# wyf-ACCEPT/BackToReality

Hardware: NVIDIA B200
Metric: Pointnet2Backbone fwd+bwd scenes/sec @40k pts (higher is better)
Workload: dtype tf32 fwd / bf16 bwd operands, f32 accumulate

## Files before the change

backtoreality_b200/csrc/mlp_bwd.cu:

```cuda
#include <cuda_bf16.h>

#include "mlp_common.cuh"

namespace b2r {
using namespace mlp;
namespace {

constexpr int kBwdWarps = 12;
constexpr int kBwdThreads = kBwdWarps * 32;

struct BwdArgs {
  int B, N, NP, NS, Cin, Cout, mode, top;
  const float *xyz, *new_xyz, *feat_t;
  const int *idx;
  float radius;
  int normalize_xyz;
  const float *z_prev, *scale_prev, *shift_prev;
  const void *w_image;
  const float *dz;
  const float *gr, *z;
  const float *dysel;
  const int *asel;
  const float *coef_a, *coef_b, *coef_c;
  float *dW;
  float *gr_prev;
  double *stats_prev;
  float *g_feat_t, *g_xyz, *g_new_xyz;
  int do_dgrad;
  int Kp, KA, WA, Cout_pad, num_tiles;
  int ch8_shift;
  int ns_shift;
  const int *cidx, *ccen, *cmeta;
};

__host__ __device__ inline int packed_k16(int Cin, int gather) {
  if (!gather) return (Cin + 7) & ~7;
  return ((Cin - 3 + 7) & ~7) + 8;
}

struct BwdSmem {
  uint32_t w_off, w_bytes, x_off[2], dz_off[2], x_bytes, dz_bytes, coef_off, scale_off, idx_off,
      cen_off, meta_off, route_off, flush_off, bar_off, total;
};
__host__ __device__ inline BwdSmem bwd_smem_layout(int Kp, int KA, int WA, int Cout, int Cout_pad,
                                                   int NT, int top, int cmp = 0) {
  BwdSmem s;
  s.w_off = 0;
  s.w_bytes = (uint32_t)Cout_pad * WA * 128u;
  s.x_bytes = (uint32_t)NT * KA * 128u;
  s.dz_bytes = (uint32_t)NT * (Cout_pad >> 6) * 128u;
  uint32_t o = s.w_bytes;
  for (int st = 0; st < 2; ++st) {
    s.x_off[st] = o;
    o += s.x_bytes;
    s.dz_off[st] = o;
    o += s.dz_bytes;
  }
  s.coef_off = o;
  s.scale_off = s.coef_off + 3u * Cout * 4u;
  s.idx_off = s.scale_off + 2u * Kp * 4u;
  s.cen_off = s.idx_off + 4u * (uint32_t)NT * 4u;
  s.meta_off = s.cen_off + (cmp ? 4u * (uint32_t)NT * 4u : 0u);
  s.route_off = (s.meta_off + (cmp ? 32u : 0u) + 15u) & ~15u;
  s.flush_off = s.route_off +
                (top ? 4u * (uint32_t)(NT / (cmp ? 8 : 16)) * Cout_pad * 4u : 0u);
  const uint32_t flush_bytes = 8u * 32u * 33u * 4u;
  if (cmp && 2u * (s.x_bytes + s.dz_bytes) >= flush_bytes) {
    s.bar_off = s.flush_off;
    s.flush_off = s.x_off[0];
  } else {
    s.bar_off = s.flush_off + flush_bytes;
  }
  s.total = s.bar_off + 13 * 8 + 16 + 1024;
  return s;
}

__device__ __forceinline__ uint32_t bf_off(int row, int chunk, int rows) {
  const int a = chunk >> 3, c = chunk & 7, g = row >> 3, r8 = row & 7;
  return (uint32_t)(((a * (rows >> 3) + g) << 10) + (r8 << 7) + ((c ^ r8) << 4));
}
__host__ __device__ constexpr uint32_t idesc_bf16(int n, int a_mn, int b_mn) {
  return (1u << 4) | (1u << 7) | (1u << 10) | ((uint32_t)a_mn << 15) | ((uint32_t)b_mn << 16) |
         ((uint32_t)(n >> 3) << 17) | ((128u >> 4) << 24);
}
__device__ __forceinline__ void umma_bf16(uint32_t d_tmem, uint64_t a_desc, uint64_t b_desc,
                                          uint32_t idesc, uint32_t accumulate) {
  asm volatile(
      "{\n\t"
      ".reg .pred p;\n\t"
      "setp.ne.b32 p, %4, 0;\n\t"
      "tcgen05.mma.cta_group::1.kind::f16 [%0], %1, %2, %3, p;\n\t"
      "}" ::"r"(d_tmem),
      "l"(a_desc), "l"(b_desc), "r"(idesc), "r"(accumulate)
      : "memory");
}
__device__ __forceinline__ void mbar_arrive(uint32_t bar) {
  asm volatile("mbarrier.arrive.shared::cta.b64 _, [%0];" ::"r"(bar) : "memory");
}
__device__ __forceinline__ uint32_t pack_bf16(float lo, float hi) {
  const __nv_bfloat162 v = __floats2bfloat162_rn(lo, hi);
  return *reinterpret_cast<const uint32_t *>(&v);
}
template <int N>
__device__ __forceinline__ void bar_named(int id) {
  asm volatile("bar.sync %0, %1;" ::"r"(id), "n"(N));
}

__global__ void pack_weight_bf16_kernel(const float *__restrict__ w, int Cout, int Cin, int gather,
                                        int Kp, int Cout_pad, int WA,
                                        __nv_bfloat16 *__restrict__ image) {
  const long long total = (long long)Cout_pad * WA * 64;
  for (long long e = (long long)blockIdx.x * blockDim.x + threadIdx.x; e < total;
       e += (long long)gridDim.x * blockDim.x) {
    const int co = (int)(e / (WA * 64)), kp = (int)(e % (WA * 64));
    float v = 0.f;
    if (co < Cout && kp < Kp) {
      int k = -1;
      if (gather) {
        const int C = Cin - 3, Cf8 = (C + 7) & ~7;
        if (kp < C) k = 3 + kp;
        else if (kp >= Cf8 && kp < Cf8 + 3) k = kp - Cf8;
      } else if (kp < Cin) {
        k = kp;
      }
      if (k >= 0) v = w[(size_t)co * Cin + k];
    }
    image[(bf_off(co, kp >> 3, Cout_pad) >> 1) + (kp & 7)] = __float2bfloat16_rn(v);
  }
}

template <int NT, int EW, int MODE, int TOP, bool CMP>
__global__ void __launch_bounds__(kBwdThreads, 1) sa_layer_bwd_kernel(const BwdArgs a) {
  constexpr int kMode = MODE;
  constexpr bool kTop = TOP != 0;
  constexpr int kRC = CMP ? NT / 8 : NT / 16;
  constexpr int kEpiThreads = EW * 32, kProdThreads = (kBwdWarps - 1 - EW) * 32;
  auto bar_epi = [] { bar_named<kEpiThreads>(1); };
  auto bar_prod = [] { bar_named<kProdThreads>(2); };
  extern __shared__ __align__(1024) uint8_t smem_raw[];
  uint8_t *base = reinterpret_cast<uint8_t *>((reinterpret_cast<uintptr_t>(smem_raw) + 1023) &
                                              ~(uintptr_t)1023);
  const BwdSmem L = bwd_smem_layout(a.Kp, a.KA, a.WA, a.Cout, a.Cout_pad, NT, kTop, CMP ? 1 : 0);
  uint8_t *s_w = base + L.w_off;
  float *s_ca = reinterpret_cast<float *>(base + L.coef_off);
  float *s_cb = s_ca + a.Cout;
  float *s_cc = s_cb + a.Cout;
  float *s_scale = reinterpret_cast<float *>(base + L.scale_off);
  float *s_shift = s_scale + a.Kp;
  int *s_idx4 = reinterpret_cast<int *>(base + L.idx_off);
  int *s_cen4 = reinterpret_cast<int *>(base + L.cen_off);
  int *s_meta = reinterpret_cast<int *>(base + L.meta_off);
  float *s_dy = reinterpret_cast<float *>(base + L.route_off);
  int *s_as = reinterpret_cast<int *>(s_dy + 2 * kRC * a.Cout_pad);
  uint64_t *s_bar = reinterpret_cast<uint64_t *>(base + L.bar_off);
  uint32_t *s_tmem = reinterpret_cast<uint32_t *>(s_bar + 13);
  auto bar = [&](int i) { return smem_u32(&s_bar[i]); };

  const int tid = threadIdx.x, warp = tid >> 5, lane = tid & 31;
  const int KA = a.KA;
  const int MTp = (KA + 1) >> 1;
  const int MTl = a.Cout_pad >> 7;
  constexpr int NCH = NT / 32;
  const bool has_coef = a.dz == nullptr;
  const int w12 = ((kTop && MTl > (a.do_dgrad ? MTp : 0)) ? MTl : (a.do_dgrad ? MTp : 0)) * NT;
  const uint32_t d3_col0 = 2u * (uint32_t)w12;
  constexpr uint32_t kTmemCols = 512;
  const long long per_scene = (long long)a.NP * a.NS;
  const int C = a.Cin - 3, Cf8 = (C + 7) & ~7;
  int num_tiles = a.num_tiles;
  if constexpr (CMP) {
    num_tiles = __ldg(a.cmeta + 8) / NT;
    if (tid < 8) s_meta[tid] = __ldg(a.cmeta + tid);
  }

  if (tid == 0) {
    for (int i = 0; i < 13; ++i)
      mbar_init(bar(i), (i == 0 || i == 1) ? (uint32_t)(kProdThreads / 32)
                        : (i == 10 || i == 11) ? (uint32_t)EW : 1u);
    asm volatile("fence.mbarrier_init.release.cluster;" ::: "memory");
  }
  if (warp == EW) tmem_alloc(smem_u32(s_tmem), kTmemCols);
  {
    const uint32_t zb = 2u * (L.x_bytes + L.dz_bytes);
    for (uint32_t i = tid * 16; i < zb; i += kBwdThreads * 16)
      *reinterpret_cast<uint4 *>(base + L.x_off[0] + i) = make_uint4(0, 0, 0, 0);
  }
  if (kMode == 1)
    for (int i = tid; i < a.Cin; i += kBwdThreads) {
      s_scale[i] = a.scale_prev[i];
      s_shift[i] = a.shift_prev[i];
    }
  if (has_coef)
    for (int i = tid; i < a.Cout; i += kBwdThreads) {
      s_ca[i] = a.coef_a[i];
      s_cb[i] = a.coef_b[i];
      s_cc[i] = a.coef_c[i];
    }
  fence_async_smem();
  tc_fence_before();
  __syncthreads();
  tc_fence_after();
  const uint32_t tmem_base = *s_tmem;
  const bool need_w = kTop || a.do_dgrad;
  if (tid == 0 && need_w) {
    mbar_expect_tx(bar(12), L.w_bytes);
    bulk_g2s(smem_u32(s_w), a.w_image, L.w_bytes, bar(12));
  }
  const int grid = (int)gridDim.x;

  if (warp > EW) {
    const int ptid = tid - (kEpiThreads + 32);
    const int CH8 = a.Cout >> 3;
    const int ch8s = (CH8 & (CH8 - 1)) == 0 ? 31 - __clz(CH8) : -1;
    const int CHx = a.Cin >> 3;
    const int chxs = (CHx > 0 && (CHx & (CHx - 1)) == 0) ? 31 - __clz(CHx) : -1;
    int nidx = 0, ncen = 0;
    for (int k = 0, tile = blockIdx.x; tile < num_tiles; tile += grid, ++k) {
      const int s = k & 1, n = k >> 1;
      mbar_wait(bar(2 + s), (uint32_t)((n & 1) ^ 1));
      const long long pos0 = (long long)tile * NT;
      uint8_t *sx = base + L.x_off[s], *sdz = base + L.dz_off[s];
      int *s_idx = s_idx4 + (k & 3) * NT;
      int *s_cen = s_cen4 + (k & 3) * NT;
      TileClass tc{};
      int p64 = 0;
      if constexpr (CMP) {
        tc = tile_class(s_meta, pos0, a.NS);
        p64 = (int)(pos0 & 63);
      }
      if (ptid == 0 && tile + 2 * grid < num_tiles) {
        const size_t pn = (size_t)(pos0 + 2ll * grid * NT);
        if (!kTop) {
          if (!has_coef) prefetch_l2(a.dz + pn * a.Cout, (uint32_t)NT * a.Cout * 4u);
          else {
            prefetch_l2(a.gr + pn * a.Cout, (uint32_t)NT * a.Cout * 4u);
            prefetch_l2(a.z + pn * a.Cout, (uint32_t)NT * a.Cout * 4u);
          }
        }
        if (kMode == 1) prefetch_l2(a.z_prev + pn * a.Cin, (uint32_t)NT * a.Cin * 4u);
      }
      if (!kTop) {
        const int total = NT * CH8;
        const size_t o0 = (size_t)pos0 * a.Cout;
        for (int i0 = ptid; i0 < total; i0 += kProdThreads * 4) {
          float4 g[4][2], zz[4][2];
#pragma unroll
          for (int u = 0; u < 4; ++u) {
            const int i = i0 + u * kProdThreads;
            if (i < total) {
              if (!has_coef) {
                const float4 *p = reinterpret_cast<const float4 *>(a.dz + o0) + 2 * i;
                g[u][0] = __ldg(p); g[u][1] = __ldg(p + 1);
              } else {
                const float4 *p = reinterpret_cast<const float4 *>(a.gr + o0) + 2 * i;
                const float4 *qz = reinterpret_cast<const float4 *>(a.z + o0) + 2 * i;
                g[u][0] = __ldg(p); g[u][1] = __ldg(p + 1);
                zz[u][0] = __ldg(qz); zz[u][1] = __ldg(qz + 1);
              }
            }
          }
#pragma unroll
          for (int u = 0; u < 4; ++u) {
            const int i = i0 + u * kProdThreads;
            if (i < total) {
              const int row = ch8s >= 0 ? (i >> ch8s) : (i / CH8), ch = i - row * CH8;
              float v[8] = {g[u][0].x, g[u][0].y, g[u][0].z, g[u][0].w,
                            g[u][1].x, g[u][1].y, g[u][1].z, g[u][1].w};
              if (has_coef) {
                const float zv[8] = {zz[u][0].x, zz[u][0].y, zz[u][0].z, zz[u][0].w,
                                     zz[u][1].x, zz[u][1].y, zz[u][1].z, zz[u][1].w};
                float ca8[8], cb8[8], cc8[8];
                *reinterpret_cast<float4 *>(ca8) = *reinterpret_cast<const float4 *>(s_ca + ch * 8);
                *reinterpret_cast<float4 *>(ca8 + 4) = *reinterpret_cast<const float4 *>(s_ca + ch * 8 + 4);
                *reinterpret_cast<float4 *>(cb8) = *reinterpret_cast<const float4 *>(s_cb + ch * 8);
                *reinterpret_cast<float4 *>(cb8 + 4) = *reinterpret_cast<const float4 *>(s_cb + ch * 8 + 4);
                *reinterpret_cast<float4 *>(cc8) = *reinterpret_cast<const float4 *>(s_cc + ch * 8);
                *reinterpret_cast<float4 *>(cc8 + 4) = *reinterpret_cast<const float4 *>(s_cc + ch * 8 + 4);
                if constexpr (CMP) {
                  const float wgt = row < tc.live
                                        ? ((((p64 + row) & (tc.ns - 1)) == 0) ? 1.f + tc.wx : 1.f)
                                        : 0.f;
#pragma unroll
                  for (int e = 0; e < 8; ++e)
                    v[e] = fmaf(ca8[e], v[e], wgt * fmaf(cb8[e], zv[e], cc8[e]));
                } else {
#pragma unroll
                  for (int e = 0; e < 8; ++e) v[e] = fmaf(ca8[e], v[e], fmaf(cb8[e], zv[e], cc8[e]));
                }
              }
              *reinterpret_cast<uint4 *>(sdz + bf_off(row, ch, NT)) =
                  make_uint4(pack_bf16(v[0], v[1]), pack_bf16(v[2], v[3]), pack_bf16(v[4], v[5]),
                             pack_bf16(v[6], v[7]));
            }
          }
        }
      }
      if (kMode == 0) {
        if constexpr (kProdThreads < NT) {
          for (int r = ptid; r < NT; r += kProdThreads) {
            if constexpr (CMP) {
              s_idx[r] = __ldg(a.cidx + pos0 + r);
              s_cen[r] = __ldg(a.ccen + pos0 + r);
            } else {
              s_idx[r] = __ldg(a.idx + pos0 + r);
            }
          }
        } else if (ptid < NT) {
          if constexpr (CMP) {
            s_idx[ptid] = (k == 0) ? a.cidx[pos0 + ptid] : nidx;
            s_cen[ptid] = (k == 0) ? a.ccen[pos0 + ptid] : ncen;
            if (tile + grid < num_tiles) {
              nidx = __ldg(a.cidx + pos0 + (long long)grid * NT + ptid);
              ncen = __ldg(a.ccen + pos0 + (long long)grid * NT + ptid);
            }
          } else {
            s_idx[ptid] = (k == 0) ? a.idx[pos0 + ptid] : nidx;
            if (tile + grid < num_tiles) nidx = __ldg(a.idx + pos0 + (long long)grid * NT + ptid);
          }
        }
        bar_prod();
        const int b = CMP ? 0 : (int)(pos0 / per_scene);
        const int in_scene0 = CMP ? 0 : (int)(pos0 - (long long)b * per_scene);
        const int CH8f = Cf8 >> 3;
        for (int row = ptid; row < NT; row += kProdThreads) {
          const int p = s_idx[row];
          const int j = CMP ? max(s_cen[row], 0) : (in_scene0 + row) / a.NS;
          const float *pp = a.xyz + ((size_t)b * a.N + p) * 3;
          const float *qq = a.new_xyz + ((size_t)b * a.NP + j) * 3;
          const float px = __ldg(pp), py = __ldg(pp + 1), pz = __ldg(pp + 2);
          const float qx = __ldg(qq), qy = __ldg(qq + 1), qz = __ldg(qq + 2);
          float d0 = __fsub_rn(px, qx), d1 = __fsub_rn(py, qy), d2 = __fsub_rn(pz, qz);
          if (a.normalize_xyz) {
            d0 = __fdiv_rn(d0, a.radius);
            d1 = __fdiv_rn(d1, a.radius);
            d2 = __fdiv_rn(d2, a.radius);
          }
          *reinterpret_cast<uint4 *>(sx + bf_off(row, CH8f, NT)) =
              make_uint4(pack_bf16(d0, d1), pack_bf16(d2, 0.f), 0u, 0u);
        }
        if (CH8f > 0) {
          const float *fb = a.feat_t + (size_t)b * a.N * C;
          const int total = NT * CH8f;
          if ((C & 7) == 0) {
            for (int i0 = ptid; i0 < total; i0 += kProdThreads * 4) {
              float4 t[4][2];
#pragma unroll
              for (int u = 0; u < 4; ++u) {
                const int i = i0 + u * kProdThreads;
                if (i < total) {
                  const int row = a.ch8_shift >= 0 ? (i >> a.ch8_shift) : (i / CH8f);
                  const int ch = i - row * CH8f;
                  const float4 *p =
                      reinterpret_cast<const float4 *>(fb + (size_t)s_idx[row] * C) + 2 * ch;
                  t[u][0] = __ldg(p); t[u][1] = __ldg(p + 1);
                }
              }
#pragma unroll
              for (int u = 0; u < 4; ++u) {
                const int i = i0 + u * kProdThreads;
                if (i < total) {
                  const int row = a.ch8_shift >= 0 ? (i >> a.ch8_shift) : (i / CH8f);
                  const int ch = i - row * CH8f;
                  *reinterpret_cast<uint4 *>(sx + bf_off(row, ch, NT)) =
                      make_uint4(pack_bf16(t[u][0].x, t[u][0].y), pack_bf16(t[u][0].z, t[u][0].w),
                                 pack_bf16(t[u][1].x, t[u][1].y), pack_bf16(t[u][1].z, t[u][1].w));
                }
              }
            }
          } else {
            for (int i = ptid; i < total; i += kProdThreads) {
              const int row = i / CH8f, ch = i - row * CH8f;
              const float *src = fb + (size_t)s_idx[row] * C + ch * 8;
              float f[8];
#pragma unroll
              for (int e = 0; e < 8; ++e) f[e] = (ch * 8 + e < C) ? __ldg(src + e) : 0.f;
              *reinterpret_cast<uint4 *>(sx + bf_off(row, ch, NT)) =
                  make_uint4(pack_bf16(f[0], f[1]), pack_bf16(f[2], f[3]), pack_bf16(f[4], f[5]),
                             pack_bf16(f[6], f[7]));
            }
          }
        }
      } else {
        const int CH = a.Cin >> 3;
        const int total = NT * CH;
        const float4 *src = reinterpret_cast<const float4 *>(a.z_prev + (size_t)pos0 * a.Cin);
        for (int i0 = ptid; i0 < total; i0 += kProdThreads * 4) {
          float4 t[4][2];
#pragma unroll
          for (int u = 0; u < 4; ++u) {
            const int i = i0 + u * kProdThreads;
            if (i < total) { t[u][0] = __ldg(src + 2 * i); t[u][1] = __ldg(src + 2 * i + 1); }
          }
#pragma unroll
          for (int u = 0; u < 4; ++u) {
            const int i = i0 + u * kProdThreads;
            if (i < total) {
              const int row = chxs >= 0 ? (i >> chxs) : (i / CH), ch = i - row * CH;
              const float *sc = s_scale + ch * 8, *sh = s_shift + ch * 8;
              const float x0 = fmaxf(fmaf(t[u][0].x, sc[0], sh[0]), 0.f);
              const float x1 = fmaxf(fmaf(t[u][0].y, sc[1], sh[1]), 0.f);
              const float x2 = fmaxf(fmaf(t[u][0].z, sc[2], sh[2]), 0.f);
              const float x3 = fmaxf(fmaf(t[u][0].w, sc[3], sh[3]), 0.f);
              const float x4 = fmaxf(fmaf(t[u][1].x, sc[4], sh[4]), 0.f);
              const float x5 = fmaxf(fmaf(t[u][1].y, sc[5], sh[5]), 0.f);
              const float x6 = fmaxf(fmaf(t[u][1].z, sc[6], sh[6]), 0.f);
              const float x7 = fmaxf(fmaf(t[u][1].w, sc[7], sh[7]), 0.f);
              *reinterpret_cast<uint4 *>(sx + bf_off(row, ch, NT)) =
                  make_uint4(pack_bf16(x0, x1), pack_bf16(x2, x3), pack_bf16(x4, x5),
                             pack_bf16(x6, x7));
            }
          }
        }
      }
      fence_async_smem();
      __syncwarp();
      if (lane == 0) mbar_arrive(bar(0 + s));
    }
  } else if (warp == EW) {
    if (lane == 0) {
      if (need_w) mbar_wait(bar(12), 0);
      const uint32_t wa = smem_u32(s_w);
      const uint32_t lbo_w = (uint32_t)(a.Cout_pad >> 3) * 1024u;
      const uint32_t lbo_t = (uint32_t)(NT >> 3) * 1024u;
      const int KS16 = (a.Kp + 15) >> 4, KSl16 = (a.Cout + 15) >> 4;
      for (int k = 0, tile = blockIdx.x; tile < num_tiles; tile += grid, ++k) {
        const int s = k & 1, n = k >> 1;
        const uint32_t xa = smem_u32(base + L.x_off[s]), dza = smem_u32(base + L.dz_off[s]);
        const uint32_t d12 = tmem_base + (uint32_t)(s * w12);
        mbar_wait(bar(0 + s), (uint32_t)(n & 1));
        mbar_wait(bar(10 + s), (uint32_t)((n & 1) ^ 1));
        tc_fence_after();
        if (kTop) {
          for (int ml = 0; ml < MTl; ++ml)
            for (int ks = 0; ks < KS16; ++ks) {
              const uint64_t ad = smem_desc_sw128(wa + (uint32_t)(ks >> 2) * lbo_w +
                                                  (uint32_t)ml * 16u * 1024u + (uint32_t)(ks & 3) * 32u);
              const uint64_t bd =
                  smem_desc_sw128(xa + (uint32_t)(ks >> 2) * lbo_t + (uint32_t)(ks & 3) * 32u);
              umma_bf16(d12 + (uint32_t)ml * NT, ad, bd, idesc_bf16(NT, 0, 0), ks > 0 ? 1u : 0u);
            }
          umma_commit(bar(4 + s));
          mbar_wait(bar(6 + s), (uint32_t)(n & 1));
          tc_fence_after();
        }
        if (a.do_dgrad) {
          for (int m = 0; m < MTp; ++m)
            for (int ks = 0; ks < KSl16; ++ks) {
              const uint64_t ad = smem_desc_sw128_mn(
                  wa + (uint32_t)(2 * m) * lbo_w + (uint32_t)ks * 2048u, lbo_w, 1024u);
              const uint64_t bd =
                  smem_desc_sw128(dza + (uint32_t)(ks >> 2) * lbo_t + (uint32_t)(ks & 3) * 32u);
              umma_bf16(d12 + (uint32_t)m * NT, ad, bd, idesc_bf16(NT, 1, 0), ks > 0 ? 1u : 0u);
            }
        }
        for (int ml = 0; ml < MTl; ++ml)
          for (int a0 = 0; a0 < KA; a0 += 4) {
            const int na = (KA - a0) < 4 ? (KA - a0) : 4;
            const uint32_t idw = idesc_bf16(na * 64, 1, 1);
            for (int k16 = 0; k16 < NT / 16; ++k16) {
              const uint64_t ad = smem_desc_sw128_mn(
                  dza + (uint32_t)(2 * ml) * lbo_t + (uint32_t)k16 * 2048u, lbo_t, 1024u);
              const uint64_t bd = smem_desc_sw128_mn(
                  xa + (uint32_t)a0 * lbo_t + (uint32_t)k16 * 2048u, lbo_t, 1024u);
              umma_bf16(tmem_base + d3_col0 + (uint32_t)(ml * KA + a0) * 64u, ad, bd, idw,
                        (k > 0 || k16 > 0) ? 1u : 0u);
            }
          }
        umma_commit(bar(8 + s));
        umma_commit(bar(2 + s));
      }
    }
    __syncwarp();
  } else {
    const int q = warp & 3, h = warp >> 2;
    const uint32_t lane_addr = (uint32_t)(q * 32) << 16;
    float s1[3] = {0.f, 0.f, 0.f}, s2[3] = {0.f, 0.f, 0.f};
    double d1[3] = {0.0, 0.0, 0.0}, d2[3] = {0.0, 0.0, 0.0};
    int ntiles = 0;
    auto fetch_route = [&](int k, int tile) {
      if (tile < num_tiles) {
        const int s = k & 1;
        const long long pos0 = (long long)tile * NT;
        int ns_t = a.NS, shift_t = a.ns_shift;
        if constexpr (CMP) {
          ns_t = tile_class(s_meta, pos0, a.NS).ns;
          shift_t = 31 - __clz(ns_t);
        }
        const long long centre0 = pos0 >> shift_t;
        const int base_s = (int)(pos0 & (ns_t - 1));
        const int ncen = ((base_s + NT - 1) >> shift_t) + 1;
        float *my_dy = s_dy + (size_t)s * kRC * a.Cout_pad;
        int *my_as = s_as + (size_t)s * kRC * a.Cout_pad;
        int cg_lane = -1;
        if constexpr (CMP) {
          if (lane < ncen) cg_lane = __ldg(a.ccen + pos0 + (lane == 0 ? 0 : lane * ns_t - base_s));
        }
        for (int c = 0; c < ncen; ++c) {
          long long cg = centre0 + c;
          if constexpr (CMP) cg = __shfl_sync(0xffffffffu, cg_lane, c);
          for (int ml = 0; ml < MTl; ++ml) {
            const int co = ml * 128 + q * 32 + lane;
            if (co < a.Cout) {
              if constexpr (CMP) {
                if (cg < 0) {
                  my_dy[c * a.Cout_pad + co] = 0.f;
                  my_as[c * a.Cout_pad + co] = -1;
                  continue;
                }
              }
              const size_t o = (size_t)cg * a.Cout + co;
              asm volatile("cp.async.ca.shared.global [%0], [%1], 4;" ::"r"(
                               smem_u32(my_dy + c * a.Cout_pad + co)),
                           "l"(a.dysel + o)
                           : "memory");
              asm volatile("cp.async.ca.shared.global [%0], [%1], 4;" ::"r"(
                               smem_u32(my_as + c * a.Cout_pad + co)),
                           "l"(a.asel + o)
                           : "memory");
            }
          }
        }
      }
      asm volatile("cp.async.commit_group;" ::: "memory");
    };
    auto produce_dz = [&](int k, int tile) {
      const int s = k & 1, n = k >> 1;
      const long long pos0 = (long long)tile * NT;
      const uint32_t d12 = tmem_base + (uint32_t)(s * w12);
      uint8_t *sdz = base + L.dz_off[s];
      TileClass tc{};
      int ns_t = a.NS, shift_t = a.ns_shift;
      if constexpr (CMP) {
        tc = tile_class(s_meta, pos0, a.NS);
        ns_t = tc.ns;
        shift_t = 31 - __clz(ns_t);
      }
      const int ns_mask = ns_t - 1;
      const int base_s = (int)(pos0 & ns_mask);
      const float *my_dy = s_dy + (size_t)s * kRC * a.Cout_pad;
      const int *my_as = s_as + (size_t)s * kRC * a.Cout_pad;
      asm volatile("cp.async.wait_group 1;" ::: "memory");
      mbar_wait(bar(4 + s), (uint32_t)(n & 1));
      tc_fence_after();
#pragma unroll
      for (int ml = 0; ml < 2; ++ml) {
        if (ml >= MTl) continue;
        const int co = ml * 128 + q * 32 + lane;
        const bool ok = co < a.Cout;
        const float ca = ok ? s_ca[co] : 0.f, cb = ok ? s_cb[co] : 0.f, cc = ok ? s_cc[co] : 0.f;
#pragma unroll
        for (int c0 = 0; c0 < NCH; c0 += (EW == 8 ? 2 : 1)) {
          const int ch = c0 + (EW == 8 ? h : 0);
          uint32_t r[32];
          cuda::ptx::tcgen05_ld_32x32b(r, d12 + lane_addr + (uint32_t)(ml * NT + ch * 32));
          asm volatile("tcgen05.wait::ld.sync.aligned;" ::: "memory");
          if (ok && CMP) {
#pragma unroll
            for (int sg = 0; sg < 4; ++sg) {
              const int colb = ch * 32 + sg * 8;
              const int t0 = base_s + colb;
              const int c = t0 >> shift_t;
              const int s0 = t0 & ns_mask;
              const float dyv = my_dy[c * a.Cout_pad + co];
              const int as = my_as[c * a.Cout_pad + co] - s0;
              const float w0 = colb < tc.live ? 1.f : 0.f;
#pragma unroll
              for (int i = 0; i < 8; ++i) {
                const float dy = (i == as) ? dyv : 0.f;
                const float wgt = (s0 + i == 0) ? w0 * (1.f + tc.wx) : w0;
                const float v =
                    fmaf(ca, dy, wgt * fmaf(cb, __uint_as_float(r[sg * 8 + i]), cc));
                *reinterpret_cast<__nv_bfloat16 *>(
                    sdz + bf_off(colb + i, co >> 3, NT) + (co & 7) * 2) = __float2bfloat16_rn(v);
              }
            }
          } else if (ok) {
#pragma unroll
            for (int hf = 0; hf < 2; ++hf) {
              const int t0 = base_s + ch * 32 + hf * 16;
              const int c = t0 >> a.ns_shift;
              const int s0 = t0 & ns_mask;
              const float dyv = my_dy[c * a.Cout_pad + co];
              const int as = my_as[c * a.Cout_pad + co] - s0;
#pragma unroll
              for (int i = 0; i < 16; ++i) {
                const float dy = (i == as) ? dyv : 0.f;
                const float v = fmaf(ca, dy, fmaf(cb, __uint_as_float(r[hf * 16 + i]), cc));
                *reinterpret_cast<__nv_bfloat16 *>(
                    sdz + bf_off(ch * 32 + hf * 16 + i, co >> 3, NT) + (co & 7) * 2) =
                    __float2bfloat16_rn(v);
              }
            }
          }
        }
      }
      tc_fence_before();
      fence_async_smem();
      bar_epi();
      if (tid == 0) mbar_arrive(bar(6 + s));
      fetch_route(k + 2, tile + 2 * grid);
    };
    if (kTop) {
      fetch_route(0, blockIdx.x);
      fetch_route(1, blockIdx.x + grid);
      if ((int)blockIdx.x < num_tiles) produce_dz(0, blockIdx.x);
    }
    for (int k = 0, tile = blockIdx.x; tile < num_tiles; tile += grid, ++k, ++ntiles) {
      const int s = k & 1, n = k >> 1;
      const long long pos0 = (long long)tile * NT;
      const uint32_t d12 = tmem_base + (uint32_t)(s * w12);
      const int *s_idx = s_idx4 + (k & 3) * NT;
      const int *s_cen = s_cen4 + (k & 3) * NT;
      if (kTop && tile + grid < num_tiles) produce_dz(k + 1, tile + grid);
      mbar_wait(bar(8 + s), (uint32_t)(n & 1));
      tc_fence_after();
      if (a.do_dgrad) {
        int tile_b = 0, in_scene0 = 0;
        if (kMode == 0 && !CMP) {
          tile_b = (int)(pos0 / per_scene);
          in_scene0 = (int)(pos0 - (long long)tile_b * per_scene);
        }
        int ns_t = a.NS;
        if constexpr (CMP) {
          if (kMode == 0) {
            ns_t = tile_class(s_meta, pos0, a.NS).ns;
            in_scene0 = (int)(pos0 & 63);
          }
        }
#pragma unroll
        for (int m = 0; m < 3; ++m) {
          if (m >= MTp) continue;
#pragma unroll
          for (int c0 = 0; c0 < NCH; c0 += (EW == 8 ? 2 : 1)) {
            const int cc = c0 + (EW == 8 ? h : 0);
            uint32_t r[32];
            cuda::ptx::tcgen05_ld_32x32b(r, d12 + lane_addr + (uint32_t)(m * NT + cc * 32));
            asm volatile("tcgen05.wait::ld.sync.aligned;" ::: "memory");
            const int kp = m * 128 + q * 32 + lane;
            const long long p0 = pos0 + cc * 32;
            if (kMode == 1) {
              if (kp < a.Cin) {
                const float sc = s_scale[kp], sh = s_shift[kp];
                const float *zp = a.z_prev + (size_t)p0 * a.Cin + kp;
                float *gp = a.gr_prev + (size_t)p0 * a.Cin + kp;
                float t1 = 0.f, t2 = 0.f;
                float zv[32];
#pragma unroll
                for (int i = 0; i < 32; ++i) zv[i] = __ldg(zp + (size_t)i * a.Cin);
#pragma unroll
                for (int i = 0; i < 32; ++i) {
                  const float g = fmaf(zv[i], sc, sh) > 0.f ? __uint_as_float(r[i]) : 0.f;
                  gp[(size_t)i * a.Cin] = g;
                  t1 += g;
                  t2 = fmaf(g, zv[i], t2);
                }
                s1[m] += t1;
                s2[m] += t2;
              }
            } else {
              const bool is_feat = kp < C;
              const int e = kp - Cf8;
              const bool is_xyz = (e >= 0 && e < 3);
              if (is_feat && a.g_feat_t != nullptr) {
                float *gb = a.g_feat_t + (size_t)tile_b * a.N * C + kp;
#pragma unroll
                for (int i = 0; i < 32; ++i)
                  atomicAdd(gb + (size_t)s_idx[cc * 32 + i] * C, __uint_as_float(r[i]));
              } else if (is_xyz && (a.g_xyz != nullptr || a.g_new_xyz != nullptr)) {
                float run = 0.f;
                float *gx = a.g_xyz != nullptr ? a.g_xyz + (size_t)tile_b * a.N * 3 + e : nullptr;
#pragma unroll
                for (int i = 0; i < 32; ++i) {
                  const int ins = in_scene0 + cc * 32 + i;
                  float v = __uint_as_float(r[i]);
                  if (a.normalize_xyz) v = __fdiv_rn(v, a.radius);
                  if (gx != nullptr) atomicAdd(gx + (size_t)s_idx[cc * 32 + i] * 3, v);
                  run += v;
                  if constexpr (CMP) {
                    if (((ins + 1) & (ns_t - 1)) == 0 || i == 31) {
                      const int cg = s_cen[cc * 32 + i];
                      if (a.g_new_xyz != nullptr && cg >= 0)
                        atomicAdd(a.g_new_xyz + (size_t)cg * 3 + e, -run);
                      run = 0.f;
                    }
                  } else if (((ins + 1) % a.NS) == 0 || i == 31) {
                    if (a.g_new_xyz != nullptr)
                      atomicAdd(a.g_new_xyz + ((size_t)tile_b * a.NP + ins / a.NS) * 3 + e, -run);
                    run = 0.f;
                  }
                }
              }
            }
          }
        }
        if (kMode == 1) {
#pragma unroll
          for (int m = 0; m < 3; ++m) {
            d1[m] += (double)s1[m];
            d2[m] += (double)s2[m];
            s1[m] = 0.f;
            s2[m] = 0.f;
          }
        }
      }
      tc_fence_before();
      __syncwarp();
      if (lane == 0) mbar_arrive(bar(10 + s));
    }

    if (a.do_dgrad && kMode == 1 && a.stats_prev != nullptr) {
#pragma unroll
      for (int m = 0; m < 3; ++m) {
        const int kp = m * 128 + q * 32 + lane;
        if (m < MTp && kp < a.Cin) {
          atomicAdd(a.stats_prev + kp, d1[m]);
          atomicAdd(a.stats_prev + a.Cin + kp, d2[m]);
        }
      }
    }
    if (ntiles > 0) {
      tc_fence_after();
      float *stg = reinterpret_cast<float *>(base + L.flush_off) + warp * (32 * 33);
      for (int ml = 0; ml < MTl; ++ml) {
        const int co0 = ml * 128 + q * 32;
        for (int at = (EW == 8 ? h : 0); at < KA * 2; at += (EW == 8 ? 2 : 1)) {
          uint32_t r[32];
          cuda::ptx::tcgen05_ld_32x32b(
              r, tmem_base + lane_addr + d3_col0 + (uint32_t)(ml * KA * 64 + at * 32));
          asm volatile("tcgen05.wait::ld.sync.aligned;" ::: "memory");
#pragma unroll
          for (int i = 0; i < 32; ++i) stg[lane * 33 + i] = __uint_as_float(r[i]);
          __syncwarp();
          const int kp = at * 32 + lane;
          int kk = -1;
          if (kMode == 0) {
            if (kp < C) kk = 3 + kp;
            else if (kp >= Cf8 && kp < Cf8 + 3) kk = kp - Cf8;
          } else if (kp < a.Cin) {
            kk = kp;
          }
          if (kk >= 0) {
            const int rows = min(32, a.Cout - co0);
            for (int rr = 0; rr < rows; ++rr)
              atomicAdd(a.dW + (size_t)(co0 + rr) * a.Cin + kk, stg[rr * 33 + lane]);
          }
          __syncwarp();
        }
      }
    }
  }
  tc_fence_before();
  __syncthreads();
  if (warp == EW) tmem_dealloc(tmem_base, kTmemCols);
}

__global__ void pool_bwd_prep_kernel(const float *__restrict__ dout_cm,
                                     const float *__restrict__ dout_pm,
                                     const float *__restrict__ zmax, const float *__restrict__ zmin,
                                     const int *__restrict__ amax, const int *__restrict__ amin,
                                     const float *__restrict__ scale,
                                     const float *__restrict__ shift, int NP, int Cch,
                                     float *__restrict__ dysel, int *__restrict__ asel,
                                     double *__restrict__ stats) {
  __shared__ float t[32][33];
  __shared__ double r1[8][32], r2[8][32];
  const int b = blockIdx.z;
  const int j0 = blockIdx.x * 32, c0 = blockIdx.y * 32;
  if (dout_cm != nullptr) {
    for (int i = threadIdx.y; i < 32; i += blockDim.y) {
      const int cc = c0 + i, j = j0 + threadIdx.x;
      t[i][threadIdx.x] = (cc < Cch && j < NP) ? dout_cm[((size_t)b * Cch + cc) * NP + j] : 0.f;
    }
    __syncthreads();
  }
  const int ch = c0 + threadIdx.x;
  const float s = ch < Cch ? scale[ch] : 0.f, sh = ch < Cch ? shift[ch] : 0.f;
  const bool pos = s >= 0.f;
  double a1 = 0.0, a2 = 0.0;
  for (int i = threadIdx.y; i < 32; i += blockDim.y) {
    const int j = j0 + i;
    if (j < NP && ch < Cch) {
      const size_t o = ((size_t)b * NP + j) * Cch + ch;
      const float zs = pos ? zmax[o] : zmin[o];
      const int as = pos ? amax[o] : amin[o];
      float g = dout_cm != nullptr ? t[threadIdx.x][i] : 0.f;
      if (dout_pm != nullptr) g += dout_pm[o];
      g = fmaf(zs, s, sh) > 0.f ? g : 0.f;
      dysel[o] = g;
      asel[o] = as;
      a1 += (double)g;
      a2 += (double)g * (double)zs;
    }
  }
  r1[threadIdx.y][threadIdx.x] = a1;
  r2[threadIdx.y][threadIdx.x] = a2;
  __syncthreads();
  if (threadIdx.y == 0 && ch < Cch) {
    for (int k = 1; k < 8; ++k) {
      a1 += r1[k][threadIdx.x];
      a2 += r2[k][threadIdx.x];
    }
    atomicAdd(stats + ch, a1);
    atomicAdd(stats + Cch + ch, a2);
  }
}

__global__ void bn_bwd_finalize_kernel(const double *__restrict__ stats, int Cch, double count,
                                       double inv_count,
                                       const float *__restrict__ gamma,
                                       const float *__restrict__ mean,
                                       const float *__restrict__ invstd, int training,
                                       float *__restrict__ coef_a, float *__restrict__ coef_b,
                                       float *__restrict__ coef_c, float *__restrict__ k1_out,
                                       float *__restrict__ k2_out, float *__restrict__ gs_out,
                                       float *__restrict__ dgamma, float *__restrict__ dbeta,
                                       float *__restrict__ dbias_conv) {
  const int ch = blockIdx.x * blockDim.x + threadIdx.x;
  if (ch >= Cch) return;
  const double S1 = stats[ch], S2 = stats[Cch + ch];
  const double mu = (double)mean[ch], is = (double)invstd[ch];
  const double g = gamma ? (double)gamma[ch] : 1.0;
  const double sx = (S2 - mu * S1) * is;
  const double gs = g * is;
  double k1 = 0.0, k2 = 0.0;
  if (training) {
    k1 = S1 * inv_count;
    k2 = sx * inv_count;
  }
  const double b = -gs * k2 * is;
  if (coef_a) coef_a[ch] = (float)gs;
  if (coef_b) coef_b[ch] = (float)b;
  if (coef_c) coef_c[ch] = (float)(-gs * k1 - b * mu);
  if (k1_out) k1_out[ch] = (float)k1;
  if (k2_out) k2_out[ch] = (float)k2;
  if (gs_out) gs_out[ch] = (float)gs;
  if (dgamma) dgamma[ch] = (float)sx;
  if (dbeta) dbeta[ch] = (float)S1;
  if (dbias_conv) dbias_conv[ch] = (float)(gs * S1 + count * (b * mu + (-gs * k1 - b * mu)));
}

}

}

using namespace b2r;

namespace {
struct Geometry {
  int Kp, KA, WA, Cout_pad;
};
Geometry bwd_geometry(int Cout, int Cin, int gather) {
  Geometry g;
  g.Kp = packed_k16(Cin, gather);
  g.KA = (g.Kp + 63) >> 6;
  const int MTp = (g.KA + 1) >> 1;
  g.WA = g.KA > 2 * MTp ? g.KA : 2 * MTp;
  g.Cout_pad = (Cout + 127) & ~127;
  return g;
}
}

namespace {
int bwd_pick_nt(const Geometry &g, int Cout, int mode, int top, int do_dgrad, int NS, long long M,
                long long per_scene, int cmp = 0) {
  const int MTp = (g.KA + 1) >> 1, MTl = g.Cout_pad >> 7;
  if (MTp > 3) return 0;
  for (int nt : {128, 64, 32}) {
    if (M % nt) continue;
    if (!cmp && mode == 0 && per_scene % nt) continue;
    if (top && (nt % NS) != 0 && (NS % nt) != 0) continue;
    const BwdSmem L = bwd_smem_layout(g.Kp, g.KA, g.WA, Cout, g.Cout_pad, nt, top, cmp);
    const int w12 = ((top && MTl > (do_dgrad ? MTp : 0)) ? MTl : (do_dgrad ? MTp : 0)) * nt;
    const int cols = 2 * w12 + MTl * g.KA * 64;
    if (L.total <= 227u * 1024u && cols <= 512) return nt;
  }
  return 0;
}
}

extern "C" int b2r_sa_layer_bwd_supported(int B, int NP, int NS, int Cin, int Cout, int gather,
                                          int top) {
  if (B <= 0 || NP <= 0 || NS <= 0 || Cin <= 0 || Cout <= 0) return 0;
  if (Cout > 256 || (Cout % 8) != 0 || (!gather && (Cin % 8) != 0) || (gather && Cin < 3)) return 0;
  if (top && pow2_shift(NS) < 0) return 0;
  const Geometry g = bwd_geometry(Cout, Cin, gather);
  const long long per_scene = (long long)NP * NS, M = (long long)B * per_scene;
  return bwd_pick_nt(g, Cout, gather ? 0 : 1, top, 1, NS, M, per_scene) > 0 ? 1 : 0;
}

extern "C" int b2r_sa_layer_bwd_tile(int B, int NP, int NS, int Cin, int Cout, int gather, int top,
                                     int dgrad, int compact) {
  if (B <= 0 || NP <= 0 || NS <= 0 || Cin <= 0 || Cout <= 0) return 0;
  const Geometry g = bwd_geometry(Cout, Cin, gather);
  const long long per_scene = (long long)NP * NS;
  const long long M = compact ? b2r_compact_capacity(B, NP, NS) : (long long)B * per_scene;
  return bwd_pick_nt(g, Cout, gather ? 0 : 1, top, dgrad, NS, M, per_scene, compact ? 1 : 0);
}

extern "C" long long b2r_mlp_weight_bf16_image_bytes(int Cout, int Cin, int gather) {
  if (Cout <= 0 || Cin <= 0) return 0;
  const Geometry g = bwd_geometry(Cout, Cin, gather);
  return (long long)g.Cout_pad * g.WA * 128;
}

extern "C" int b2r_mlp_pack_weight_bf16(const float *w, int Cout, int Cin, int gather, void *image,
                                        void *stream) {
  B2R_REQUIRE(w && image && Cout > 0 && Cin > 0, "b2r_mlp_pack_weight_bf16: bad argument");
  B2R_REQUIRE(!gather || Cin >= 3, "b2r_mlp_pack_weight_bf16: gather layers need Cin >= 3");
  const Geometry g = bwd_geometry(Cout, Cin, gather);
  const long long total = (long long)g.Cout_pad * g.WA * 64;
  pack_weight_bf16_kernel<<<ceil_div(total, 256), 256, 0, static_cast<cudaStream_t>(stream)>>>(
      w, Cout, Cin, gather, g.Kp, g.Cout_pad, g.WA, static_cast<__nv_bfloat16 *>(image));
  B2R_CHECK_LAUNCH();
  return B2R_OK;
}

extern "C" int b2r_sa_layer_bwd(const b2r_sa_layer_bwd_desc *d, void *stream) {
  B2R_REQUIRE(d != nullptr, "b2r_sa_layer_bwd: null descriptor");
  B2R_REQUIRE(d->B > 0 && d->NP > 0 && d->NS > 0 && d->Cin > 0 && d->Cout > 0,
              "b2r_sa_layer_bwd: non-positive size");
  B2R_REQUIRE(d->mode == 0 || d->mode == 1, "b2r_sa_layer_bwd: mode must be 0 or 1");
  B2R_REQUIRE(d->dW != nullptr, "b2r_sa_layer_bwd: null dW");
  const bool top = d->dysel != nullptr;
  B2R_REQUIRE(d->dz != nullptr || (d->coef_a && d->coef_b && d->coef_c &&
                                   ((d->gr && d->z) || (top && d->asel))),
              "b2r_sa_layer_bwd: needs dz, or gr + z + coef_a/b/c, or dysel + asel + coef_a/b/c");
  BwdArgs a;
  a.B = d->B; a.N = d->N; a.NP = d->NP; a.NS = d->NS; a.Cin = d->Cin; a.Cout = d->Cout;
  a.mode = d->mode;
  a.top = (d->dz == nullptr && top) ? 1 : 0;
  a.xyz = d->xyz; a.new_xyz = d->new_xyz; a.feat_t = d->feat_t; a.idx = d->idx;
  a.radius = d->radius; a.normalize_xyz = d->normalize_xyz;
  a.z_prev = d->z_prev; a.scale_prev = d->scale_prev; a.shift_prev = d->shift_prev;
  a.w_image = d->w_image_bf16;
  a.dz = d->dz; a.gr = d->gr; a.z = d->z; a.dysel = d->dysel; a.asel = d->asel;
  a.coef_a = d->coef_a; a.coef_b = d->coef_b; a.coef_c = d->coef_c;
  a.dW = d->dW; a.gr_prev = d->gr_prev; a.stats_prev = d->stats_prev;
  a.g_feat_t = d->g_feat_t; a.g_xyz = d->g_xyz; a.g_new_xyz = d->g_new_xyz;
  const Geometry g = bwd_geometry(d->Cout, d->Cin, d->mode == 0);
  a.Kp = g.Kp; a.KA = g.KA; a.WA = g.WA; a.Cout_pad = g.Cout_pad;
  a.ch8_shift = pow2_shift((((d->Cin - 3 + 7) & ~7) >> 3));
  a.ns_shift = pow2_shift(d->NS);
  a.cidx = d->cidx; a.ccen = d->ccen; a.cmeta = d->cmeta;
  const int cmp = d->cmeta != nullptr ? 1 : 0;
  B2R_REQUIRE(!cmp || (d->cidx && d->ccen), "b2r_sa_layer_bwd: a plan needs cidx, ccen and cmeta");
  if (cmp && !(d->NS == 16 || d->NS == 32 || d->NS == 64)) {
    set_error("b2r_sa_layer_bwd: a compacted plan needs nsample 16/32/64 (got %d)", d->NS);
    return B2R_ERR_UNSUPPORTED;
  }
  if (a.top && a.ns_shift < 0) {
    set_error("b2r_sa_layer_bwd: the pooled top layer needs a power-of-two nsample (got %d)", d->NS);
    return B2R_ERR_UNSUPPORTED;
  }
  a.num_tiles = 0;
  if (d->mode == 0) {
    B2R_REQUIRE(d->Cin >= 3 && d->xyz && d->new_xyz && (d->idx || cmp) && (d->feat_t || d->Cin == 3),
                "b2r_sa_layer_bwd: gather mode needs xyz, new_xyz, idx (and feat_t when Cin > 3)");
    a.do_dgrad = (d->g_feat_t != nullptr && d->Cin > 3) || d->g_xyz != nullptr ||
                 d->g_new_xyz != nullptr;
  } else {
    B2R_REQUIRE(d->z_prev && d->scale_prev && d->shift_prev,
                "b2r_sa_layer_bwd: dense mode needs z_prev/scale/shift");
    B2R_REQUIRE(d->gr_prev != nullptr, "b2r_sa_layer_bwd: dense mode needs gr_prev");
    a.do_dgrad = 1;
  }
  B2R_REQUIRE(!(a.do_dgrad || a.top) || d->w_image_bf16 != nullptr,
              "b2r_sa_layer_bwd: null weight image");
  if (thin::bwd_applicable(d)) return thin::bwd_launch(d, stream);
  const long long M = cmp ? b2r_compact_capacity(d->B, d->NP, d->NS)
                          : (long long)d->B * d->NP * d->NS;
  const long long per_scene = (long long)d->NP * d->NS;
  if (a.Cout_pad > 256 || (d->Cout % 8) != 0 || (d->mode == 1 && (d->Cin % 8) != 0)) {
    set_error("b2r_sa_layer_bwd: needs Cout %% 8 == 0, Cout <= 256, dense Cin %% 8 == 0 "
              "(Cin=%d Cout=%d)", d->Cin, d->Cout);
    return B2R_ERR_UNSUPPORTED;
  }
  const int NT = bwd_pick_nt(g, d->Cout, d->mode, a.top, a.do_dgrad, d->NS, M, per_scene, cmp);
  if (NT == 0) {
    set_error("b2r_sa_layer_bwd: layer Cin=%d Cout=%d M=%lld does not fit shared memory / TMEM",
              d->Cin, d->Cout, M);
    return B2R_ERR_UNSUPPORTED;
  }
  const BwdSmem L = bwd_smem_layout(a.Kp, a.KA, a.WA, a.Cout, a.Cout_pad, NT, a.top, cmp);
  a.num_tiles = (int)(M / NT);
  int sms = kNumSMs;
  if (d->sm_limit > 0 && d->sm_limit < kNumSMs) sms = d->sm_limit;
  const int grid = a.num_tiles < sms ? a.num_tiles : sms;
  cudaStream_t st = static_cast<cudaStream_t>(stream);
#define B2R_LAUNCH_BWD2(NTV, EWV, MV, TV, CV)                                                   \
  do {                                                                                          \
    B2R_CUDA(cudaFuncSetAttribute(sa_layer_bwd_kernel<NTV, EWV, MV, TV, CV>,                    \
                                  cudaFuncAttributeMaxDynamicSharedMemorySize, (int)L.total));  \
    sa_layer_bwd_kernel<NTV, EWV, MV, TV, CV><<<grid, kBwdThreads, L.total, st>>>(a);           \
  } while (0)
#define B2R_LAUNCH_BWD1(NTV, EWV, MV, TV)                                                       \
  do {                                                                                          \
    if (cmp) B2R_LAUNCH_BWD2(NTV, EWV, MV, TV, true); else B2R_LAUNCH_BWD2(NTV, EWV, MV, TV, false); \
  } while (0)
#define B2R_LAUNCH_BWD(NTV, EWTOP)                                                              \
  do {                                                                                          \
    if (a.top) {                                                                                \
      if (a.mode == 0) B2R_LAUNCH_BWD1(NTV, EWTOP, 0, 1); else B2R_LAUNCH_BWD1(NTV, EWTOP, 1, 1); \
    } else {                                                                                    \
      if (a.mode == 0) B2R_LAUNCH_BWD1(NTV, 4, 0, 0); else B2R_LAUNCH_BWD1(NTV, 4, 1, 0);       \
    }                                                                                           \
  } while (0)
  if (NT == 128) B2R_LAUNCH_BWD(128, 8);
  else if (NT == 64) B2R_LAUNCH_BWD(64, 8);
  else B2R_LAUNCH_BWD(32, 4);
#undef B2R_LAUNCH_BWD
#undef B2R_LAUNCH_BWD1
#undef B2R_LAUNCH_BWD2
  B2R_CHECK_LAUNCH();
  return B2R_OK;
}

extern "C" int b2r_pool_bwd_prep(const float *dout_cm, const float *dout_pm, const float *zmax,
                                 const float *zmin, const int *amax, const int *amin,
                                 const float *scale, const float *shift, int B, int NP, int C,
                                 float *dysel, int *asel, double *stats, void *stream) {
  B2R_REQUIRE((dout_cm || dout_pm) && zmax && zmin && amax && amin && scale && shift && dysel &&
                  asel && stats && B > 0 && NP > 0 && C > 0 && C <= 1024,
              "b2r_pool_bwd_prep: bad argument");
  B2R_REQUIRE(B <= 65535, "b2r_pool_bwd_prep: B=%d exceeds gridDim.z", B);
  dim3 grid(ceil_div(NP, 32), ceil_div(C, 32), B), block(32, 8);
  pool_bwd_prep_kernel<<<grid, block, 0, static_cast<cudaStream_t>(stream)>>>(
      dout_cm, dout_pm, zmax, zmin, amax, amin, scale, shift, NP, C, dysel, asel, stats);
  B2R_CHECK_LAUNCH();
  return B2R_OK;
}

extern "C" int b2r_bn_bwd_finalize_ex(const double *stats, int C, double count, const float *gamma,
                                      const float *mean, const float *invstd, int training,
                                      float *coef_a, float *coef_b, float *coef_c, float *k1,
                                      float *k2, float *gs, float *dgamma, float *dbeta,
                                      float *dbias_conv, void *stream) {
  B2R_REQUIRE(stats && mean && invstd && C > 0 && count > 0, "b2r_bn_bwd_finalize: bad argument");
  bn_bwd_finalize_kernel<<<ceil_div(C, 128), 128, 0, static_cast<cudaStream_t>(stream)>>>(
      stats, C, count, 1.0 / count, gamma, mean, invstd, training, coef_a, coef_b, coef_c, k1, k2, gs, dgamma,
      dbeta, dbias_conv);
  B2R_CHECK_LAUNCH();
  return B2R_OK;
}

extern "C" int b2r_bn_bwd_finalize(const double *stats, int C, double count, const float *gamma,
                                   const float *mean, const float *invstd, int training,
                                   float *coef_a, float *coef_b, float *coef_c, float *k1,
                                   float *k2, float *gs, float *dgamma, float *dbeta,
                                   void *stream) {
  return b2r_bn_bwd_finalize_ex(stats, C, count, gamma, mean, invstd, training, coef_a, coef_b,
                                coef_c, k1, k2, gs, dgamma, dbeta, nullptr, stream);
}
```

Measured before the change: 2436.

## Use TMEM slot ring for dgrad accumulators in non-top backward layers

```diff
diff --git a/backtoreality_b200/csrc/mlp_bwd.cu b/backtoreality_b200/csrc/mlp_bwd.cu
--- a/backtoreality_b200/csrc/mlp_bwd.cu
+++ b/backtoreality_b200/csrc/mlp_bwd.cu
@@ -31,7 +31,13 @@
   int ch8_shift;
   int ns_shift;
   const int *cidx, *ccen, *cmeta;
+  int ring;
 };
+
+constexpr int kMaxRing = 8;
+constexpr int kBarSlotFull = 13, kBarSlotFree = kBarSlotFull + kMaxRing;
+constexpr int kBarDone = kBarSlotFree + kMaxRing, kNumBars = kBarDone + 1;
+constexpr int kIdxBufs = 8;
 
 __host__ __device__ inline int packed_k16(int Cin, int gather) {
   if (!gather) return (Cin + 7) & ~7;
@@ -59,19 +65,19 @@
   s.coef_off = o;
   s.scale_off = s.coef_off + 3u * Cout * 4u;
   s.idx_off = s.scale_off + 2u * Kp * 4u;
-  s.cen_off = s.idx_off + 4u * (uint32_t)NT * 4u;
-  s.meta_off = s.cen_off + (cmp ? 4u * (uint32_t)NT * 4u : 0u);
+  s.cen_off = s.idx_off + kIdxBufs * (uint32_t)NT * 4u;
+  s.meta_off = s.cen_off + (cmp ? kIdxBufs * (uint32_t)NT * 4u : 0u);
   s.route_off = (s.meta_off + (cmp ? 32u : 0u) + 15u) & ~15u;
   s.flush_off = s.route_off +
                 (top ? 4u * (uint32_t)(NT / (cmp ? 8 : 16)) * Cout_pad * 4u : 0u);
   const uint32_t flush_bytes = 8u * 32u * 33u * 4u;
-  if (cmp && 2u * (s.x_bytes + s.dz_bytes) >= flush_bytes) {
+  if (2u * (s.x_bytes + s.dz_bytes) >= flush_bytes) {
     s.bar_off = s.flush_off;
     s.flush_off = s.x_off[0];
   } else {
     s.bar_off = s.flush_off + flush_bytes;
   }
-  s.total = s.bar_off + 13 * 8 + 16 + 1024;
+  s.total = s.bar_off + kNumBars * 8 + 16 + 1024;
   return s;
 }
 
@@ -147,13 +153,13 @@
   float *s_cc = s_cb + a.Cout;
   float *s_scale = reinterpret_cast<float *>(base + L.scale_off);
   float *s_shift = s_scale + a.Kp;
-  int *s_idx4 = reinterpret_cast<int *>(base + L.idx_off);
-  int *s_cen4 = reinterpret_cast<int *>(base + L.cen_off);
+  int *s_idx_r = reinterpret_cast<int *>(base + L.idx_off);
+  int *s_cen_r = reinterpret_cast<int *>(base + L.cen_off);
   int *s_meta = reinterpret_cast<int *>(base + L.meta_off);
   float *s_dy = reinterpret_cast<float *>(base + L.route_off);
   int *s_as = reinterpret_cast<int *>(s_dy + 2 * kRC * a.Cout_pad);
   uint64_t *s_bar = reinterpret_cast<uint64_t *>(base + L.bar_off);
-  uint32_t *s_tmem = reinterpret_cast<uint32_t *>(s_bar + 13);
+  uint32_t *s_tmem = reinterpret_cast<uint32_t *>(s_bar + kNumBars);
   auto bar = [&](int i) { return smem_u32(&s_bar[i]); };
 
   const int tid = threadIdx.x, warp = tid >> 5, lane = tid & 31;
@@ -163,7 +169,7 @@
   constexpr int NCH = NT / 32;
   const bool has_coef = a.dz == nullptr;
   const int w12 = ((kTop && MTl > (a.do_dgrad ? MTp : 0)) ? MTl : (a.do_dgrad ? MTp : 0)) * NT;
-  const uint32_t d3_col0 = 2u * (uint32_t)w12;
+  const uint32_t d3_col0 = kTop ? 2u * (uint32_t)w12 : (uint32_t)(a.ring * NT);
   constexpr uint32_t kTmemCols = 512;
   const long long per_scene = (long long)a.NP * a.NS;
   const int C = a.Cin - 3, Cf8 = (C + 7) & ~7;
@@ -174,9 +180,10 @@
   }
 
   if (tid == 0) {
-    for (int i = 0; i < 13; ++i)
+    for (int i = 0; i < kNumBars; ++i)
       mbar_init(bar(i), (i == 0 || i == 1) ? (uint32_t)(kProdThreads / 32)
-                        : (i == 10 || i == 11) ? (uint32_t)EW : 1u);
+                        : (i == 10 || i == 11 || (i >= kBarSlotFree && i < kBarDone)) ? (uint32_t)EW
+                                                                                      : 1u);
     asm volatile("fence.mbarrier_init.release.cluster;" ::: "memory");
   }
   if (warp == EW) tmem_alloc(smem_u32(s_tmem), kTmemCols);
@@ -220,8 +227,8 @@
       mbar_wait(bar(2 + s), (uint32_t)((n & 1) ^ 1));
       const long long pos0 = (long long)tile * NT;
       uint8_t *sx = base + L.x_off[s], *sdz = base + L.dz_off[s];
-      int *s_idx = s_idx4 + (k & 3) * NT;
-      int *s_cen = s_cen4 + (k & 3) * NT;
+      int *s_idx = s_idx_r + (k & (kIdxBufs - 1)) * NT;
+      int *s_cen = s_cen_r + (k & (kIdxBufs - 1)) * NT;
       TileClass tc{};
       int p64 = 0;
       if constexpr (CMP) {
@@ -423,12 +430,13 @@
       const uint32_t lbo_w = (uint32_t)(a.Cout_pad >> 3) * 1024u;
       const uint32_t lbo_t = (uint32_t)(NT >> 3) * 1024u;
       const int KS16 = (a.Kp + 15) >> 4, KSl16 = (a.Cout + 15) >> 4;
+      int slot = 0, slot_ph = 0;
       for (int k = 0, tile = blockIdx.x; tile < num_tiles; tile += grid, ++k) {
         const int s = k & 1, n = k >> 1;
         const uint32_t xa = smem_u32(base + L.x_off[s]), dza = smem_u32(base + L.dz_off[s]);
         const uint32_t d12 = tmem_base + (uint32_t)(s * w12);
         mbar_wait(bar(0 + s), (uint32_t)(n & 1));
-        mbar_wait(bar(10 + s), (uint32_t)((n & 1) ^ 1));
+        if (kTop) mbar_wait(bar(10 + s), (uint32_t)((n & 1) ^ 1));
         tc_fence_after();
         if (kTop) {
           for (int ml = 0; ml < MTl; ++ml)
@@ -444,14 +452,25 @@
           tc_fence_after();
         }
         if (a.do_dgrad) {
-          for (int m = 0; m < MTp; ++m)
+          for (int m = 0; m < MTp; ++m) {
+            uint32_t d2 = d12 + (uint32_t)m * NT;
+            if (!kTop) {
+              mbar_wait(bar(kBarSlotFree + slot), (uint32_t)(slot_ph ^ 1));
+              tc_fence_after();
+              d2 = tmem_base + (uint32_t)(slot * NT);
+            }
             for (int ks = 0; ks < KSl16; ++ks) {
               const uint64_t ad = smem_desc_sw128_mn(
                   wa + (uint32_t)(2 * m) * lbo_w + (uint32_t)ks * 2048u, lbo_w, 1024u);
               const uint64_t bd =
                   smem_desc_sw128(dza + (uint32_t)(ks >> 2) * lbo_t + (uint32_t)(ks & 3) * 32u);
-              umma_bf16(d12 + (uint32_t)m * NT, ad, bd, idesc_bf16(NT, 1, 0), ks > 0 ? 1u : 0u);
-            }
+              umma_bf16(d2, ad, bd, idesc_bf16(NT, 1, 0), ks > 0 ? 1u : 0u);
+            }
+            if (!kTop) {
+              umma_commit(bar(kBarSlotFull + slot));
+              if (++slot == a.ring) { slot = 0; slot_ph ^= 1; }
+            }
+          }
         }
         for (int ml = 0; ml < MTl; ++ml)
           for (int a0 = 0; a0 < KA; a0 += 4) {
@@ -466,9 +485,10 @@
                         (k > 0 || k16 > 0) ? 1u : 0u);
             }
           }
-        umma_commit(bar(8 + s));
+        if (kTop) umma_commit(bar(8 + s));
         umma_commit(bar(2 + s));
       }
+      umma_commit(bar(kBarDone));
     }
     __syncwarp();
   } else {
@@ -605,15 +625,18 @@
       fetch_route(1, blockIdx.x + grid);
       if ((int)blockIdx.x < num_tiles) produce_dz(0, blockIdx.x);
     }
+    int slot = 0, slot_ph = 0;
     for (int k = 0, tile = blockIdx.x; tile < num_tiles; tile += grid, ++k, ++ntiles) {
       const int s = k & 1, n = k >> 1;
       const long long pos0 = (long long)tile * NT;
       const uint32_t d12 = tmem_base + (uint32_t)(s * w12);
-      const int *s_idx = s_idx4 + (k & 3) * NT;
-      const int *s_cen = s_cen4 + (k & 3) * NT;
+      const int *s_idx = s_idx_r + (k & (kIdxBufs - 1)) * NT;
+      const int *s_cen = s_cen_r + (k & (kIdxBufs - 1)) * NT;
       if (kTop && tile + grid < num_tiles) produce_dz(k + 1, tile + grid);
-      mbar_wait(bar(8 + s), (uint32_t)(n & 1));
-      tc_fence_after();
+      if (kTop) {
+        mbar_wait(bar(8 + s), (uint32_t)(n & 1));
+        tc_fence_after();
+      }
       if (a.do_dgrad) {
         int tile_b = 0, in_scene0 = 0;
         if (kMode == 0 && !CMP) {
@@ -630,12 +653,24 @@
 #pragma unroll
         for (int m = 0; m < 3; ++m) {
           if (m >= MTp) continue;
+          uint32_t d2 = d12 + (uint32_t)m * NT;
+          if (!kTop) {
+            mbar_wait(bar(kBarSlotFull + slot), (uint32_t)slot_ph);
+            tc_fence_after();
+            d2 = tmem_base + (uint32_t)(slot * NT);
+          }
 #pragma unroll
           for (int c0 = 0; c0 < NCH; c0 += (EW == 8 ? 2 : 1)) {
             const int cc = c0 + (EW == 8 ? h : 0);
             uint32_t r[32];
-            cuda::ptx::tcgen05_ld_32x32b(r, d12 + lane_addr + (uint32_t)(m * NT + cc * 32));
+            cuda::ptx::tcgen05_ld_32x32b(r, d2 + lane_addr + (uint32_t)(cc * 32));
             asm volatile("tcgen05.wait::ld.sync.aligned;" ::: "memory");
+            if (!kTop && c0 + (EW == 8 ? 2 : 1) >= NCH) {
+              tc_fence_before();
+              __syncwarp();
+              if (lane == 0) mbar_arrive(bar(kBarSlotFree + slot));
+              if (++slot == a.ring) { slot = 0; slot_ph ^= 1; }
+            }
             const int kp = m * 128 + q * 32 + lane;
             const long long p0 = pos0 + cc * 32;
             if (kMode == 1) {
@@ -703,9 +738,11 @@
           }
         }
       }
-      tc_fence_before();
-      __syncwarp();
-      if (lane == 0) mbar_arrive(bar(10 + s));
+      if (kTop) {
+        tc_fence_before();
+        __syncwarp();
+        if (lane == 0) mbar_arrive(bar(10 + s));
+      }
     }
 
     if (a.do_dgrad && kMode == 1 && a.stats_prev != nullptr) {
@@ -719,6 +756,7 @@
       }
     }
     if (ntiles > 0) {
+      mbar_wait(bar(kBarDone), 0u);
       tc_fence_after();
       float *stg = reinterpret_cast<float *>(base + L.flush_off) + warp * (32 * 33);
       for (int ml = 0; ml < MTl; ++ml) {
@@ -861,6 +899,12 @@
 }
 
 namespace {
+int bwd_ring(const Geometry &g, int nt) {
+  const int MTp = (g.KA + 1) >> 1, d3_cols = (g.Cout_pad >> 7) * g.KA * 64;
+  const int r = (512 - d3_cols) / nt;
+  return r < 2 * MTp ? r : 2 * MTp;
+}
+
 int bwd_pick_nt(const Geometry &g, int Cout, int mode, int top, int do_dgrad, int NS, long long M,
                 long long per_scene, int cmp = 0) {
   const int MTp = (g.KA + 1) >> 1, MTl = g.Cout_pad >> 7;
@@ -871,8 +915,16 @@
     if (top && (nt % NS) != 0 && (NS % nt) != 0) continue;
     const BwdSmem L = bwd_smem_layout(g.Kp, g.KA, g.WA, Cout, g.Cout_pad, nt, top, cmp);
     const int w12 = ((top && MTl > (do_dgrad ? MTp : 0)) ? MTl : (do_dgrad ? MTp : 0)) * nt;
-    const int cols = 2 * w12 + MTl * g.KA * 64;
-    if (L.total <= 227u * 1024u && cols <= 512) return nt;
+    const int d3_cols = MTl * g.KA * 64;
+    const bool tmem_ok = top ? 2 * w12 + d3_cols <= 512
+                             : (!do_dgrad || bwd_ring(g, nt) >= MTp) && d3_cols <= 512;
+    if (!(L.total <= 227u * 1024u && tmem_ok)) continue;
+    if (!top && do_dgrad && nt > 32 && bwd_ring(g, nt) < 2 * MTp) {
+      const long long busiest = (M / nt + kNumSMs - 1) / kNumSMs * nt;
+      const long long busiest_half = (M / (nt / 2) + kNumSMs - 1) / kNumSMs * (nt / 2);
+      if (busiest > busiest_half) continue;
+    }
+    return nt;
   }
   return 0;
 }
@@ -982,6 +1034,7 @@
     return B2R_ERR_UNSUPPORTED;
   }
   const BwdSmem L = bwd_smem_layout(a.Kp, a.KA, a.WA, a.Cout, a.Cout_pad, NT, a.top, cmp);
+  a.ring = (!a.top && a.do_dgrad) ? bwd_ring(g, NT) : 0;
   a.num_tiles = (int)(M / NT);
   int sms = kNumSMs;
   if (d->sm_limit > 0 && d->sm_limit < kNumSMs) sms = d->sm_limit;
```

After: 2440, median of 6. No clear change (+0.2%).
